# wangyunpeng139/3_ORB_SLAM3_SelfNote

Measured on AMD Instinct MI355X. Metric: frames/sec ORB extract+match, 752x480, higher is better.
Workload: dtype u8; 1 GPU; BASELINE configs[2]: extract + SearchByProjection match, 1000x1000 candidates, synthetic frame stream; image=752x480, nfeatures=1000, nlevels=8, batch=256, distinct_frames_per_gpu=2048, streams=4

## Files before the change

### 3_orb_slam3_selfnote_amd/csrc/orb_kernels.h

```cpp
#pragma once
#include <hip/hip_runtime.h>
#include <type_traits>
#include "orb_common.h"
#include "orb_fast_score.h"
#include "orb_sincos.h"

#define WAVE 64

__constant__ __attribute__((aligned(16))) int8_t c_pattern[1024] = {
#include "../../include/orb_pattern_data.inc"
};

struct DiscTab { uint32_t w[64][6]; };
constexpr DiscTab make_disc_tab() {
  DiscTab t{};
  const int umax[16] = {15, 15, 15, 15, 14, 14, 14, 13, 13, 12, 11, 10, 9, 8, 6, 3};
  int n = 0;
  for (int v = -15; v <= 15; v++) {
    const int d = umax[v < 0 ? -v : v];
    for (int u = -d; u <= d; u++) {
      const int lane = n & 63, k = n >> 6;
      t.w[lane][k >> 2] |= (uint32_t)(uint8_t)(int8_t)u << (8 * (k & 3));
      t.w[lane][3 + (k >> 2)] |= (uint32_t)(uint8_t)(int8_t)v << (8 * (k & 3));
      n++;
    }
  }
  return t;
}
__constant__ __attribute__((aligned(16))) DiscTab c_disc = make_disc_tab();

__device__ __forceinline__ int reflect101(int p, int n) {
  if (n == 1) return 0;
  while (p < 0 || p >= n) p = p < 0 ? -p : 2 * (n - 1) - p;
  return p;
}

__device__ __forceinline__ const uint8_t *level_plane(const FrameParams &P, int frame, int level, int &pitch) {
  if (level == 0) {
    pitch = (int)P.img0_stride;
    return P.img0 + (size_t)frame * P.img0_frame_stride;
  }
  pitch = P.geom[level].pitch;
  return P.pyr + (size_t)frame * P.pyr_fs + P.geom[level].off;
}

__device__ __forceinline__ void xcd_map(int nitems, uint32_t magic, int nframes, int &frame, int &item) {
  const unsigned b = blockIdx.x;
  const unsigned full = (unsigned)(nframes & ~7);
  const unsigned nfull = full * (unsigned)nitems;
  const bool inFull = b < nfull;
  const unsigned q = inFull ? (b >> 3) : (b - nfull);
  unsigned g = __umulhi(q, magic);
  unsigned r = q - g * (unsigned)nitems;
  if (r >= (unsigned)nitems) { g++; r -= (unsigned)nitems; }
  frame = (int)(inFull ? (b & 7u) + 8u * g : full + g);
  item = (int)r;
}

template <int CTRL, int ROWMASK>
__device__ __forceinline__ int dpp_or_zero(int v) { return __builtin_amdgcn_update_dpp(0, v, CTRL, ROWMASK, 0xf, false); }
__device__ __forceinline__ uint32_t mul24(uint32_t a, uint32_t u) {
  uint32_t d;
  asm("v_mul_u32_u24 %0, %1, %2" : "=v"(d) : "s"(u), "v"(a));
  return d;
}
__device__ __forceinline__ uint32_t mul24_vv(uint32_t a, uint32_t b) { return __umul24(a, b); }

__device__ __forceinline__ int wave_sum_i32(int v) {
  v += dpp_or_zero<0x111, 0xf>(v);
  v += dpp_or_zero<0x112, 0xf>(v);
  v += dpp_or_zero<0x114, 0xf>(v);
  v += dpp_or_zero<0x118, 0xf>(v);
  v += dpp_or_zero<0x142, 0xa>(v);
  v += dpp_or_zero<0x143, 0xc>(v);
  return __builtin_amdgcn_readlane(v, 63);
}

__device__ __forceinline__ uint32_t wave_incl_scan(uint32_t x) {
  int v = (int)x;
  v += dpp_or_zero<0x111, 0xf>(v);
  v += dpp_or_zero<0x112, 0xf>(v);
  v += dpp_or_zero<0x114, 0xf>(v);
  v += dpp_or_zero<0x118, 0xf>(v);
  v += dpp_or_zero<0x142, 0xa>(v);
  v += dpp_or_zero<0x143, 0xc>(v);
  return (uint32_t)v;
}

template <int NT>
__device__ uint32_t lds_excl_scan(uint32_t *a, int n, uint32_t *sw) {
  const int tid = threadIdx.x, lane = tid & 63, wid = tid >> 6;
  constexpr int NW = NT / 64;
  uint32_t carry = 0;
  for (int base = 0; base < n; base += NT) {
    int i = base + tid;
    uint32_t v = i < n ? a[i] : 0u;
    uint32_t inc = wave_incl_scan(v);
    if (lane == 63) sw[wid] = inc;
    __syncthreads();
    const uint32_t wsum = lane < NW ? sw[lane] : 0u;
    const uint32_t wincl = wave_incl_scan(wsum);
    const int widu = __builtin_amdgcn_readfirstlane(wid);
    const uint32_t woff = (uint32_t)__builtin_amdgcn_readlane((int)(wincl - wsum), widu);
    const uint32_t tot = (uint32_t)__builtin_amdgcn_readlane((int)wincl, NW - 1);
    if (i < n) a[i] = carry + woff + inc - v;
    carry += tot;
    __syncthreads();
  }
  return carry;
}

#define RESIZE_ROWS_MAX 16
#define RESIZE_MAXSRC 32
__global__ __launch_bounds__(256) void k_resize(FrameParams P, int level, int smemRowBytes, int tPitch, int maxSrc) {
  extern __shared__ __align__(16) uint8_t smem_rs[];
  const LevelGeom G = P.geom[level];
  const LevelGeom Gs = P.geom[level - 1];
  const int tid = threadIdx.x;
  int frame, rowTile;
  xcd_map((G.h + G.resizeRows - 1) / G.resizeRows, G.rowTileMagic, P.nframes, frame, rowTile);
  const int dy0 = rowTile * G.resizeRows;
  const int nrows = min(G.resizeRows, G.h - dy0);
  int spitch;
  const uint8_t *src = level_plane(P, frame, level - 1, spitch);
  uint8_t *dstplane = P.pyr + (size_t)frame * P.pyr_fs + G.off;
  const int wq = (G.w + 3) & ~3, qw = wq >> 2;
  __shared__ int2 sY[RESIZE_ROWS_MAX];
  if (tid < nrows) sY[tid] = P.ytab[G.ytabBase + dy0 + tid];

  if (tPitch > 0) {
    const int syFirst = min(max(P.ytab[G.ytabBase + dy0].x, 0), Gs.h - 1);
    const int syLast = min(max(P.ytab[G.ytabBase + dy0 + nrows - 1].x + 1, 0), Gs.h - 1);
    const int nsrc = min(syLast - syFirst + 1, maxSrc);
    uint8_t *sRows = smem_rs;
    uint8_t *sT = sRows + (size_t)maxSrc * smemRowBytes;
    uint4 *sRowRec = reinterpret_cast<uint4 *>(sT + (((size_t)maxSrc * tPitch + 15) & ~(size_t)15));
    const int4 *xtab4 = reinterpret_cast<const int4 *>(P.xtab + G.xtabBase);
    int4 xtPre[2];
#pragma unroll
    for (int k = 0; k < 2; k++) { const int p = tid + 256 * k; xtPre[k] = 2 * p < wq ? xtab4[p] : make_int4(0, 0, 0, 0); }
    const bool aligned = ((((uintptr_t)src) | (uintptr_t)spitch) & 3u) == 0;
    const uint8_t *src0 = src + (size_t)syFirst * spitch;
    if (aligned) {
      const int cpr = smemRowBytes >> 4, nfull = Gs.w >> 4;
      const float inv_cpr = 1.0f / (float)cpr;
      for (int idx = tid; idx < cpr * nsrc; idx += 256) {
        const int r = (int)(((float)idx + 0.5f) * inv_cpr), c = idx - (int)mul24((uint32_t)r, (uint32_t)cpr);
        if (c < nfull)
          __builtin_amdgcn_global_load_lds((const __attribute__((address_space(1))) void *)(src0 + (mul24((uint32_t)r, (uint32_t)spitch) + 16u * (uint32_t)c)),
                                           (__attribute__((address_space(3))) void *)(sRows + (size_t)(idx - (tid & 63)) * 16), 16, 0, 0);
      }
      const int ndw = (Gs.w + 3) >> 2, d0 = 4 * nfull, ntail = ndw - d0;
      const bool lastRowPartial = (Gs.w & 3) != 0;
      for (int idx = tid; idx < ntail * nsrc; idx += 256) {
        const int r = idx / ntail, d = d0 + (idx - r * ntail);
        const uint8_t *rowp = src0 + mul24((uint32_t)r, (uint32_t)spitch);
        uint32_t v;
        if (lastRowPartial && d == ndw - 1 && syFirst + r == Gs.h - 1 && spitch < 4 * ndw) {
          v = 0;
          for (int b = 0; 4 * d + b < Gs.w; b++) v |= (uint32_t)rowp[4 * d + b] << (8 * b);
        } else {
          v = *reinterpret_cast<const uint32_t *>(rowp + 4 * d);
        }
        *reinterpret_cast<uint32_t *>(sRows + mul24((uint32_t)r, (uint32_t)smemRowBytes) + 4 * d) = v;
      }
    } else {
      const float inv_w = 1.0f / (float)Gs.w;
      for (int idx = tid; idx < Gs.w * nsrc; idx += 256) {
        const int r = (int)(((float)idx + 0.5f) * inv_w), c = idx - (int)mul24((uint32_t)r, (uint32_t)Gs.w);
        sRows[mul24((uint32_t)r, (uint32_t)smemRowBytes) + c] = src0[mul24((uint32_t)r, (uint32_t)spitch) + c];
      }
    }
    if (tid < nrows) {
      const int2 yt = P.ytab[G.ytabBase + dy0 + tid];
      const int sy0 = min(max(yt.x, 0), Gs.h - 1), sy1 = min(max(yt.x + 1, 0), Gs.h - 1);
      sRowRec[tid] = make_uint4((uint32_t)((sy0 - syFirst) * tPitch), (uint32_t)((sy1 - syFirst) * tPitch), (uint32_t)yt.y, (uint32_t)((dy0 + tid) * G.pitch));
    }
    __syncthreads();
    typedef unsigned short u16x2 __attribute__((ext_vector_type(2)));
    auto dot2 = [](uint32_t pix, uint32_t coef) -> uint32_t {
      u16x2 x, y;
      __builtin_memcpy(&x, &pix, 4); __builtin_memcpy(&y, &coef, 4);
      return __builtin_amdgcn_udot2(x, y, 0u, false);
    };
    int trip = 0;
    for (int p = tid; 2 * p < wq; p += 256, trip++) {
      const int4 xt = trip == 0 ? xtPre[0] : trip == 1 ? xtPre[1] : xtab4[p];
      const uint32_t base = (uint32_t)xt.x & ~3u, oA = (uint32_t)xt.x & 3u, oB = (uint32_t)xt.z - base;
      const uint32_t selA = 0x0c000c00u | oA | ((oA + 1u) << 16), selB = 0x0c000c00u | oB | ((oB + 1u) << 16);
      const uint32_t kA = (uint32_t)xt.y << 4, kB = (uint32_t)xt.w << 4;
      const uint8_t *sp = sRows + base;
      uint8_t *tp = sT + 4 * p;
      for (int r = 0; r < nsrc; r += 4) {
        uint32_t lo[4], hi[4];
#pragma unroll
        for (int k = 0; k < 4; k++) {
          const uint32_t *q = reinterpret_cast<const uint32_t *>(sp + min(r + k, nsrc - 1) * smemRowBytes);
          lo[k] = q[0]; hi[k] = q[1];
        }
#pragma unroll
        for (int k = 0; k < 4; k++)
          if (r + k < nsrc) {
            const uint32_t vA = dot2(__builtin_amdgcn_perm(hi[k], lo[k], selA), kA), vB = dot2(__builtin_amdgcn_perm(hi[k], lo[k], selB), kB);
            *reinterpret_cast<uint32_t *>(tp + (r + k) * tPitch) = __builtin_amdgcn_perm(vB, vA, 0x06050201u);
          }
      }
    }
    __syncthreads();
    for (int ry = tid >> 5; ry < nrows; ry += 8) {
      const uint4 rec = sRowRec[ry];
      const uint32_t b0 = rec.z & 0xffffu, b1 = rec.z >> 16;
      const uint8_t *T0 = sT + rec.x, *T1 = sT + rec.y;
      uint8_t *dst = dstplane + rec.w;
      for (int qx = tid & 31; qx < qw; qx += 32) {
        const uint2 t0 = *reinterpret_cast<const uint2 *>(T0 + 8 * qx), t1 = *reinterpret_cast<const uint2 *>(T1 + 8 * qx);
        const uint32_t u0[4] = {t0.x & 0xffffu, t0.x >> 16, t0.y & 0xffffu, t0.y >> 16};
        const uint32_t u1[4] = {t1.x & 0xffffu, t1.x >> 16, t1.y & 0xffffu, t1.y >> 16};
        uint32_t packed = 0;
#pragma unroll
        for (int j = 0; j < 4; j++) {
          const uint32_t v = ((mul24_vv(b0, u0[j]) >> 16) + (mul24_vv(b1, u1[j]) >> 16) + 2) >> 2;
          packed |= v << (8 * j);
        }
        const int dx0 = 4 * qx;
        if (dx0 + 3 < G.w) *reinterpret_cast<uint32_t *>(dst + dx0) = packed;
        else for (int j = 0; j < 4 && dx0 + j < G.w; j++) dst[dx0 + j] = (uint8_t)(packed >> (8 * j));
      }
    }
    return;
  }

  int2 *sX = reinterpret_cast<int2 *>(smem_rs);
  for (int i = tid; i < wq; i += 256) sX[i] = P.xtab[G.xtabBase + i];
  __syncthreads();
  const float inv_qw = 1.0f / (float)qw;
  for (int q = tid; q < qw * nrows; q += 256) {
    const int ry = (int)(((float)q + 0.5f) * inv_qw), dx0 = (q - (int)mul24((uint32_t)ry, (uint32_t)qw)) * 4, dy = dy0 + ry;
    const int2 yt = sY[ry];
    const int sy0 = min(max(yt.x, 0), Gs.h - 1), sy1 = min(max(yt.x + 1, 0), Gs.h - 1);
    const int b0 = yt.y & 0xffff, b1 = (yt.y >> 16) & 0xffff;
    const uint8_t *S0 = src + mul24((uint32_t)sy0, (uint32_t)spitch), *S1 = src + mul24((uint32_t)sy1, (uint32_t)spitch);
    uint32_t packed = 0;
#pragma unroll
    for (int j = 0; j < 4; j++) {
      const int2 xt = sX[dx0 + j];
      const int sx = xt.x, sx1 = min(sx + 1, Gs.w - 1);
      const int a0 = xt.y & 0xffff, a1 = (xt.y >> 16) & 0xffff;
      const int r0 = S0[sx] * a0 + S0[sx1] * a1;
      const int r1 = S1[sx] * a0 + S1[sx1] * a1;
      const int v = (((b0 * (r0 >> 4)) >> 16) + ((b1 * (r1 >> 4)) >> 16) + 2) >> 2;
      packed |= (uint32_t)v << (8 * j);
    }
    uint8_t *dst = dstplane + mul24((uint32_t)dy, (uint32_t)G.pitch);
    if (dx0 + 3 < G.w) *reinterpret_cast<uint32_t *>(dst + dx0) = packed;
    else for (int j = 0; j < 4 && dx0 + j < G.w; j++) dst[dx0 + j] = (uint8_t)(packed >> (8 * j));
  }
}

__global__ __launch_bounds__(CHAIN_NT) void k_pyramid_chain(FrameParams P) {
  extern __shared__ __align__(16) uint8_t smem_ch[];
  const int tid = threadIdx.x, lane = tid & 63, wid = tid >> 6;
  constexpr int NW = CHAIN_NT / 64;
  const int ntile = (int)gridDim.x / P.nframes;
  const int frame = (int)blockIdx.x / ntile, tile = (int)blockIdx.x - frame * ntile;
  __shared__ ChainTile T;
  static_assert(sizeof(ChainTile) % 4 == 0 && sizeof(ChainTile) / 4 <= CHAIN_NT, "one dword per thread");
  if (tid < (int)(sizeof(ChainTile) / 4)) reinterpret_cast<uint32_t *>(&T)[tid] = reinterpret_cast<const uint32_t *>(&P.chain[tile])[tid];
  __syncthreads();
  const int L = T.level;
  uint8_t *buf[2] = {smem_ch, smem_ch + P.chainBuf0};
  int2 *sTab = reinterpret_cast<int2 *>(smem_ch + P.chainBuf0 + P.chainBuf1);
  {
    int off = 0;
    for (int l = 1; l <= L; l++) {
      const LevelGeom &G = P.geom[l];
      for (int i = tid; i < T.w[l] + T.h[l]; i += CHAIN_NT)
        sTab[off + i] = i < T.w[l] ? P.xtab[G.xtabBase + T.x[l] + i] : P.ytab[G.ytabBase + T.y[l] + (i - T.w[l])];
      off += T.w[l] + T.h[l];
    }
  }
  {
    const uint8_t *img = P.img0 + (size_t)frame * P.img0_frame_stride + (size_t)T.y[0] * P.img0_stride + T.x[0];
    const int rw = T.w[0], rh = T.h[0];
    for (int r = wid; r < rh; r += NW)
      for (int c = lane; c < rw; c += 64) buf[0][r * rw + c] = img[(size_t)r * P.img0_stride + c];
  }
  __syncthreads();
  int toff = 0;
  for (int l = 1; l <= L; l++) {
    const LevelGeom &G = P.geom[l];
    const LevelGeom &Gs = P.geom[l - 1];
    const int rw = T.w[l], rh = T.h[l], sw = T.w[l - 1], sx0 = T.x[l - 1], sy0 = T.y[l - 1];
    const uint8_t *S = buf[(l - 1) & 1];
    uint8_t *D = buf[l & 1];
    const int2 *sX = sTab + toff, *sY = sX + rw;
    toff += rw + rh;
    uint8_t *plane = P.pyr + (size_t)frame * P.pyr_fs + G.off + (size_t)T.y[l] * G.pitch + T.x[l];
    const float inv_rw = 1.0f / (float)rw;
    for (int idx = tid; idx < rw * rh; idx += CHAIN_NT) {
      const int ry = (int)(((float)idx + 0.5f) * inv_rw), rx = idx - ry * rw;
      const int2 xt = sX[rx], yt = sY[ry];
      const int sx = xt.x, sx1 = min(sx + 1, Gs.w - 1);
      const int sya = min(max(yt.x, 0), Gs.h - 1), syb = min(max(yt.x + 1, 0), Gs.h - 1);
      const int a0 = xt.y & 0xffff, a1 = (xt.y >> 16) & 0xffff, b0 = yt.y & 0xffff, b1 = (yt.y >> 16) & 0xffff;
      const uint8_t *S0 = S + (sya - sy0) * sw - sx0, *S1 = S + (syb - sy0) * sw - sx0;
      const int r0 = S0[sx] * a0 + S0[sx1] * a1;
      const int r1 = S1[sx] * a0 + S1[sx1] * a1;
      const int v = (((b0 * (r0 >> 4)) >> 16) + ((b1 * (r1 >> 4)) >> 16) + 2) >> 2;
      if (l == L) plane[(size_t)ry * G.pitch + rx] = (uint8_t)v;
      else D[idx] = (uint8_t)v;
    }
    __syncthreads();
  }
}

__device__ __forceinline__ int lane_rank(unsigned long long b) {
  return (int)__builtin_amdgcn_mbcnt_hi((uint32_t)(b >> 32), __builtin_amdgcn_mbcnt_lo((uint32_t)b, 0u));
}

__device__ __forceinline__ int fast_compass_sign(const uint8_t *c, int t) {
  constexpr int Pt = FAST_TILE_PITCH;
  const int v = c[0];
  const uint16_t p0 = c[3 * Pt], p4 = c[3], p8 = c[-3 * Pt], p12 = c[-3];
  const int D = (int)(uint16_t)max((uint16_t)min(p0, p8), (uint16_t)min(p4, p12));
  const int B = (int)(uint16_t)min((uint16_t)max(p0, p8), (uint16_t)max(p4, p12));
  return (D - (v - t)) | ((v + t) - B);
}

#ifndef FAST_NT
#define FAST_NT 256
#endif
#define FAST_QUEUE 128
#ifndef FAST_LIST
#define FAST_LIST 384
#endif
static_assert(FAST_NT == 4 * WAVE, "k_fast gives each cell of a 2 x 2 group a wavefront of its own");
static_assert(FAST_LIST % WAVE == 0, "pass 3 reads the corner list 64 entries at a time, all inside the list");
static_assert((FAST_TILE_ROWS * FAST_TILE_PITCH) % 16 == 0, "the score plane is cleared in 16-byte stores");
static_assert(FAST_TILE_ROWS * FAST_TILE_PITCH <= 65536, "queue entries are 16-bit tile offsets");
#if defined(FAST_STAMPS) || defined(OCT_STAMPS)
__device__ unsigned int *g_fast_stamps;
#endif
#ifdef FAST_STAMPS
#define FSTAMP(i) do { const long long t_ = __builtin_readcyclecounter(); if (threadIdx.x == 0 && g_fast_stamps) g_fast_stamps[(size_t)blockIdx.x * 8 + (i)] = (unsigned int)(t_ - ft0); ft0 = t_; } while (0)
#else
#define FSTAMP(i) do {} while (0)
#endif
__device__ __forceinline__ void wave_lds_order() {
  __builtin_amdgcn_wave_barrier();
  asm volatile("" ::: "memory");
}
__global__ __launch_bounds__(FAST_NT) void k_fast(FrameParams P) {
#ifdef FAST_STAMPS
  long long ft0 = __builtin_readcyclecounter();
#endif
  __shared__ __align__(16) uint8_t sTile[FAST_TILE_ROWS * FAST_TILE_PITCH];
  __shared__ __align__(16) uint8_t sS[FAST_TILE_ROWS * FAST_TILE_PITCH];
  __shared__ uint16_t sQ[4 * FAST_QUEUE];
  __shared__ uint16_t sL[4 * FAST_LIST];
  const int tid = threadIdx.x, lane = tid & 63;
  int groupId, frame;
  xcd_map(P.totalGroups, P.magicGroups, P.nframes, frame, groupId);
  const uint4 gr = reinterpret_cast<const uint4 *>(P.groups)[groupId];
  const int firstCell = (int)gr.x, gx = (int)(gr.y & 0xffu), gy = (int)((gr.y >> 8) & 0xffu), gStride = (int)(gr.y >> 16);
  const int tileX = (int)(gr.z & 0xffffu), tileY = (int)(gr.z >> 16);
  const int gtw = (int)(gr.w & 0xffu), gth = (int)((gr.w >> 8) & 0xffu), level = (int)((gr.w >> 16) & 0xffu);
  const bool gvalid = (gr.w >> 24) != 0u;
  const int ax = tileX & ~3;
  if (gvalid) {
    const uint4 r1f = reinterpret_cast<const uint4 *>(P.cells)[2 * firstCell + 1];
    int pitch;
    const uint8_t *img;
    if (level == 0) { pitch = (int)P.img0_stride; img = P.img0 + (size_t)frame * P.img0_frame_stride; }
    else { pitch = (int)r1f.y; img = P.pyr + (size_t)frame * P.pyr_fs + (((size_t)r1f.w << 32) | r1f.z); }
    const bool aligned = ((((uintptr_t)img) | (uintptr_t)pitch) & 3u) == 0;
    if (aligned) {
      const int nch = 5 * gth;
      const uint8_t *img0 = img + mul24((uint32_t)tileY, (uint32_t)pitch) + ax;
      for (int idx = tid; idx < nch; idx += FAST_NT) {
// ... 1157 lines not shown
```

### 3_orb_slam3_selfnote_amd/csrc/orbhip.hip

```cpp
#include <hip/hip_runtime.h>
#include <math.h>
#include <stdio.h>
#include <stdlib.h>
#include <string.h>
#include <string>
#include <vector>
#include <algorithm>
#include <type_traits>
#include <mutex>
#include <chrono>

#include "../../include/orbhip.h"
#include "orb_kernels.h"
#include "orb_match_kernels.h"
#include "orb_match_mfma.h"
#include "orb_project_kernels.h"
#include "orb_stereo_kernels.h"

static_assert(sizeof(orbx_keypoint_t) == 28, "cv::KeyPoint layout");
static_assert(sizeof(KpOut) == 28, "cv::KeyPoint layout");

namespace {

inline int cv_round(double v) { return (int)lrint(v); }
// ... 479 lines not shown
          ChainTile T;
          memset(&T, 0, sizeof(T));
          T.level = (uint16_t)L;
          int x0 = tx, x1 = std::min(tx + CHAIN_TILE, g[L].w) - 1, y0 = ty, y1 = std::min(ty + CHAIN_TILE, g[L].h) - 1;
          size_t tab = 0;
          for (int l = L; l >= 0; l--) {
            T.x[l] = (uint16_t)x0; T.y[l] = (uint16_t)y0; T.w[l] = (uint16_t)(x1 - x0 + 1); T.h[l] = (uint16_t)(y1 - y0 + 1);
            const size_t area = (size_t)T.w[l] * T.h[l];
            if (l < L) { if (l & 1) b1 = std::max(b1, area); else b0 = std::max(b0, area); }
            if (l == 0) break;
            tab += (size_t)T.w[l] + T.h[l];
            const int sw = g[l - 1].w, sh = g[l - 1].h;
            const int2 *xt = &xtab[g[l].xtabBase], *yt = &ytab[g[l].ytabBase];
            int nx0 = sw, nx1 = 0, ny0 = sh, ny1 = 0;
            for (int x = x0; x <= x1; x++) { nx0 = std::min(nx0, xt[x].x); nx1 = std::max(nx1, std::min(xt[x].x + 1, sw - 1)); }
            for (int y = y0; y <= y1; y++) {
              ny0 = std::min(ny0, std::min(std::max(yt[y].x, 0), sh - 1));
              ny1 = std::max(ny1, std::min(std::max(yt[y].x + 1, 0), sh - 1));
            }
            x0 = nx0; x1 = nx1; y0 = ny0; y1 = ny1;
          }
          tabMax = std::max(tabMax, tab);
          tilesC.push_back(T);
        }
    b0 = align_up(b0, 16); b1 = align_up(b1, 16);
    const size_t lds = b0 + b1 + sizeof(int2) * tabMax;
    h->chainTiles = 0;
    if (!tilesC.empty() && lds <= 64 * 1024 && b1 <= 16384 && b0 <= 65536 && tilesC.size() < 65536) {
      bool ok = true;
      for (const ChainTile &T : tilesC)
        for (int l = 1; l <= T.level; l++) ok = ok && (size_t)T.w[l] * T.h[l] < 16384;
      if (ok) {
        XCHECK(h, h->d_chain.reserve(sizeof(ChainTile) * tilesC.size()));
        XCHECK(h, copy_on(h->stream, h->d_chain.p, tilesC.data(), sizeof(ChainTile) * tilesC.size(), hipMemcpyHostToDevice));
        h->chainTiles = (int)tilesC.size(); h->chainBuf0 = (int)b0; h->chainBuf1 = (int)b1; h->chainLds = lds;
      }
    }
  }
  int maxCells = 1;
  for (int l = 0; l < nl; l++) maxCells = std::max(maxCells, g[l].nCols * g[l].nRows);
  size_t lds = 72 * (size_t)octCap + 128;
  if (lds > 160 * 1024 - 256) { h->err = "nfeatures too large for the LDS-resident octree"; return ORBX_E_ARG; }
  h->octCellsLds = lds + 4 * ((size_t)maxCells + 1) <= 96 * 1024;
  if (h->octCellsLds) lds += 4 * ((size_t)maxCells + 1);
  h->octLds = lds;
  if (lds > ORB_LDS_LIMIT) { h->err = "octree LDS state exceeds 160 KiB"; return ORBX_E_ARG; }
  h->rows = rows;
  h->cols = cols;
  h->max_batch = max_batch;
  h->have_last = false;
  return h->maxKeypoints;
}

void orbx_set_profiling(orbx_t *h, int enable) {
  if (!h) return;
  h->profiling = enable != 0;
  h->prof_head = 0;
  h->stage_valid = false;
  if (h->profiling && !h->ev_ok) {
    (void)hipSetDevice(h->device);
    bool ok = true;
    for (auto &set : h->ev)
      for (auto &e : set) ok = ok && hipEventCreate(&e) == hipSuccess;
    h->ev_ok = ok;
  }
}

int orbx_get_stage_ms(orbx_t *h, float *ms, int cap) {
  if (!h || !ms || !h->profiling || !h->ev_ok || !h->stage_valid || h->prof_head <= 0) return 0;
  const int nb = std::min(h->prof_head, PROF_DEPTH), n = std::min(cap, 5);
  if (hipEventSynchronize(h->ev[(h->prof_head - 1) % PROF_DEPTH][5]) != hipSuccess) return 0;
  for (int i = 0; i < n; i++) ms[i] = 0.f;
  for (int b = 0; b < nb; b++) {
    const int slot = (h->prof_head - 1 - b) % PROF_DEPTH;
    for (int i = 0; i < n; i++) {
      float t = 0;
      if (hipEventElapsedTime(&t, h->ev[slot][i], h->ev[slot][i + 1]) != hipSuccess) return 0;
      ms[i] += t / (float)nb;
    }
  }
  return n;
}

int orbx_extract_batch_device(orbx_t *h, const uint8_t *d_images, int rows, int cols, size_t stride, size_t frame_stride,
                              int nframes, int lap0, int lap1, orbx_keypoint_t *d_kps, uint8_t *d_desc, int32_t *d_counts,
                              int cap, void *stream_) {
  if (!h) return ORBX_E_ARG;
  if (!d_images || rows <= 0 || cols <= 0 || nframes <= 0) return ORBX_E_EMPTY;
  if (!d_kps || !d_desc || !d_counts || cap <= 0 || stride < (size_t)cols) return ORBX_E_ARG;
  int rc = orbx_configure(h, rows, cols, std::max(nframes, h->rows == rows && h->cols == cols ? h->max_batch : 1));
  if (rc < 0) return rc;
  if (cap < h->maxKeypoints) { h->err = "cap below orbx_configure()'s bound"; return ORBX_E_CAP; }
  XCHECK(h, hipSetDevice(h->device));
  hipStream_t s = (hipStream_t)stream_;
  FrameParams P;
  memset(&P, 0, sizeof(P));
  for (int l = 0; l < h->nlevels; l++) P.geom[l] = h->geom[l];
  P.nlevels = h->nlevels;
  P.nframes = nframes;
  P.iniTh = h->iniThFAST;
  P.minTh = h->minThFAST;
  P.lap0 = lap0;
  P.lap1 = lap1;
  P.img0 = d_images;
  P.img0_stride = stride;
  P.img0_frame_stride = frame_stride;
  P.pyr = (uint8_t *)h->d_pyr.p;       P.pyr_fs = h->pyr_fs;
  P.blur = (uint8_t *)h->d_blur.p;     P.blur_fs = h->blur_fs;
  P.cellCnt = (uint32_t *)h->d_cellCnt.p; P.cell_fs = h->cell_fs;
  P.slots = (uint32_t *)h->d_slots.p;  P.slot_fs = h->slot_fs;
  P.cand = (uint32_t *)h->d_cand.p;    P.cand_fs = h->cand_fs;
  P.knode = (uint16_t *)h->d_knode.p;
  P.lkp = (uint32_t *)h->d_lkp.p;      P.lkp_fs = h->lkp_fs;
  P.lrank = (uint16_t *)h->d_lrank.p;
  P.lcnt = (int32_t *)h->d_lcnt.p;
  P.candCnt = (int32_t *)h->d_candCnt.p;
  P.xtab = (const int2 *)h->d_xtab.p;
  P.ytab = (const int2 *)h->d_ytab.p;
  P.disc = (const int8_t *)h->d_disc.p;
  P.totalTiles = h->totalTiles;
  P.totalCells = h->totalCells;
  P.cells = (const uint32_t *)h->d_cells.p;
  P.groups = (const uint32_t *)h->d_groups.p;
  P.totalGroups = h->totalGroups;
  P.magicGroups = magic_div((uint32_t)std::max(h->totalGroups, 1));
  P.tiles = (const uint32_t *)h->d_tiles.p;
  P.magicCells = magic_div((uint32_t)std::max(h->totalCells, 1));
  P.magicTiles = magic_div((uint32_t)std::max(h->totalTiles, 1));
  const bool wide = (long long)h->nlevels * nframes <= 32;
  const int describeGroups = wide ? ORB_DESCRIBE_GROUPS(h->totalKp, 1) : ORB_DESCRIBE_GROUPS(h->totalKp, ORB_DESCRIBE_K);
  P.magicKpBlk = magic_div((uint32_t)describeGroups);
  P.totalKp = h->totalKp;
  P.octCap = h->octCap;
  P.chain = (const ChainTile *)h->d_chain.p; P.chainBuf0 = h->chainBuf0; P.chainBuf1 = h->chainBuf1;
  P.out_kps = d_kps;
  P.out_desc = d_desc;
  P.out_counts = d_counts;
  P.cap = cap;
  const bool prof = h->profiling && h->ev_ok;
  hipEvent_t *pev = h->ev[h->prof_head % PROF_DEPTH];
  if (prof) XCHECK(h, hipEventRecord(pev[0], s));
  const bool printForms = getenv("ORBHIP_PRINT_EXTRACT_FORMS") != nullptr;
  std::string pyrForm = h->nlevels == 1 ? "none" : "";
  if (wide && h->chainTiles > 0) { hipLaunchKernelGGL(k_pyramid_chain, dim3(h->chainTiles * nframes), dim3(CHAIN_NT), h->chainLds, s, P); pyrForm = "chain"; }
  else
  for (int l = 1; l < h->nlevels; l++) {
    const LevelGeom &G = h->geom[l], &Gs = h->geom[l - 1];
    const int rowBytes = (int)align_up((size_t)Gs.w + 4, 16);
    const int wq = (G.w + 3) & ~3;
    const int tPitch2 = (int)align_up((size_t)wq * 2, 8);
    const size_t lds2 = (size_t)G.resizeSrcRows * rowBytes + align_up((size_t)G.resizeSrcRows * tPitch2, 16) + 16 * RESIZE_ROWS_MAX;
    const bool twoPass = G.resizeSrcRows <= RESIZE_MAXSRC && (double)Gs.w / G.w < 3.0 && lds2 <= ORB_LDS_LIMIT - 1024;
    const int tPitch = twoPass ? tPitch2 : 0;
    const size_t lds = twoPass ? lds2 : (size_t)wq * 8;
    hipLaunchKernelGGL(k_resize, dim3(((G.h + G.resizeRows - 1) / G.resizeRows) * nframes), dim3(256), lds, s, P, l, rowBytes, tPitch, G.resizeSrcRows);
    if (printForms) pyrForm += std::string(l > 1 ? "," : "") + (!twoPass ? "1p" : G.resizeRows == 16 ? "2p16" : "2p8");
  }
  if (prof) XCHECK(h, hipEventRecord(pev[1], s));
  if (h->totalGroups > 0) hipLaunchKernelGGL(k_fast, dim3(h->totalGroups * nframes), dim3(FAST_NT), 0, s, P);
  if (prof) XCHECK(h, hipEventRecord(pev[2], s));
  if (wide) {
    if (h->octCellsLds) hipLaunchKernelGGL((k_octree<1024, true>), dim3(h->nlevels * nframes), dim3(1024), h->octLds, s, P, (uint32_t *)h->d_cellOff.p);
    else hipLaunchKernelGGL((k_octree<1024, false>), dim3(h->nlevels * nframes), dim3(1024), h->octLds, s, P, (uint32_t *)h->d_cellOff.p);
  } else {
    if (h->octCellsLds) hipLaunchKernelGGL((k_octree<256, true>), dim3(h->nlevels * nframes), dim3(256), h->octLds, s, P, (uint32_t *)h->d_cellOff.p);
    else hipLaunchKernelGGL((k_octree<256, false>), dim3(h->nlevels * nframes), dim3(256), h->octLds, s, P, (uint32_t *)h->d_cellOff.p);
  }
  if (prof) XCHECK(h, hipEventRecord(pev[3], s));
  hipLaunchKernelGGL(k_blur, dim3(h->totalTiles * nframes), dim3(256), 0, s, P);
  if (prof) XCHECK(h, hipEventRecord(pev[4], s));
  if (wide) hipLaunchKernelGGL(k_describe<1>, dim3(describeGroups * nframes), dim3(256), 0, s, P);
  else hipLaunchKernelGGL(k_describe<ORB_DESCRIBE_K>, dim3(describeGroups * nframes), dim3(256), 0, s, P);
  if (prof) { XCHECK(h, hipEventRecord(pev[5], s)); h->prof_head++; h->stage_valid = true; }
  XCHECK(h, hipGetLastError());
  if (printForms) {
    int aligned0 = 0;
    for (int f = 0; f < nframes; f++) aligned0 += (((uintptr_t)(d_images + (size_t)f * frame_stride) | (uintptr_t)stride) & 3u) == 0;
    const LevelGeom &G0 = h->geom[0];
    const int blur0dma = G0.w >= 160 && G0.h >= 40 && (G0.w & 15) == 0 ? aligned0 : 0;
    fprintf(stderr, "orbhip: extract nframes %d pyramid %s octree %d/%s aligned0 %d blur0dma %d describe %d\n", nframes, pyrForm.c_str(), wide ? 1024 : 256,
            h->octCellsLds ? "lds" : "global", aligned0, blur0dma, wide ? 1 : ORB_DESCRIBE_K);
  }
  h->last = P;
  h->have_last = true;
  if (!h->in_capture) {
    if (!h->last_done) XCHECK(h, hipEventCreateWithFlags(&h->last_done, hipEventDisableTiming));
    XCHECK(h, hipEventRecord(h->last_done, s));
    h->last_pending = true;
  }
  return 0;
}

int orbx_extract(orbx_t *h, const uint8_t *image, int rows, int cols, size_t stride, int lap0, int lap1,
                 orbx_keypoint_t *keypoints, uint8_t *descriptors, int cap, int *n_out) {
  if (!h) return ORBX_E_ARG;
  if (n_out) *n_out = 0;
  if (!image || rows <= 0 || cols <= 0) return ORBX_E_EMPTY;
  if (stride < (size_t)cols || !n_out) return ORBX_E_ARG;
  int rc = orbx_configure(h, rows, cols, h->rows == rows && h->cols == cols ? h->max_batch : 1);
  if (rc < 0) return rc;
  const int icap = h->maxKeypoints;
  const size_t dstride = align_up((size_t)cols, 64);
  XCHECK(h, hipSetDevice(h->device));
  XCHECK(h, h->d_img.reserve(dstride * rows));
  const size_t in_bytes = dstride * rows, kp_bytes = sizeof(orbx_keypoint_t) * (size_t)icap, de_bytes = 32 * (size_t)icap;
  const size_t kp_off = 64, de_off = kp_off + align_up(kp_bytes, 64), out_bytes = de_off + de_bytes;
  XCHECK(h, h->d_okps.reserve(out_bytes));
  if (h->pin_in_bytes < in_bytes) {
    if (h->pin_in) (void)hipHostFree(h->pin_in);
    h->pin_in = nullptr; h->pin_in_bytes = 0;
    XCHECK(h, hipHostMalloc(&h->pin_in, in_bytes, hipHostMallocDefault));
    h->pin_in_bytes = in_bytes;
  }
  if (h->pin_out_bytes < out_bytes) {
    if (h->pin_out) (void)hipHostFree(h->pin_out);
    h->pin_out = nullptr; h->pin_out_bytes = 0;
    XCHECK(h, hipHostMalloc(&h->pin_out, out_bytes, hipHostMallocDefault));
    h->pin_out_bytes = out_bytes;
  }
  const auto t0 = std::chrono::steady_clock::now();
  for (int y = 0; y < rows; y++) memcpy((uint8_t *)h->pin_in + (size_t)y * dstride, image + (size_t)y * stride, (size_t)cols);
  const auto t1 = std::chrono::steady_clock::now();
  uint8_t *po = (uint8_t *)h->pin_out;
  auto enqueue = [&]() -> int {
    XCHECK(h, hipMemcpyAsync(h->d_img.p, h->pin_in, in_bytes, hipMemcpyHostToDevice, h->stream));
    uint8_t *dout = (uint8_t *)h->d_okps.p;
    const int r = orbx_extract_batch_device(h, (const uint8_t *)h->d_img.p, rows, cols, dstride, dstride * rows, 1, lap0, lap1,
                                            (orbx_keypoint_t *)(dout + kp_off), dout + de_off, (int32_t *)dout, icap, h->stream);
    if (r < 0) return r;
    XCHECK(h, hipMemcpyAsync(po, dout, out_bytes, hipMemcpyDeviceToHost, h->stream));
    return 0;
  };
  bool launched = false;
  if (h->graph_ok && !h->profiling) {
    auto &K = h->graph_key;
    const bool same = h->graph && K.rows == rows && K.cols == cols && K.lap0 == lap0 && K.lap1 == lap1 && K.icap == icap && K.pin_in == h->pin_in &&
                      K.pin_out == h->pin_out && K.d_img == h->d_img.p && K.d_okps == h->d_okps.p && K.d_pyr == h->d_pyr.p;
    if (!same) {
      if (h->graph) { (void)hipGraphExecDestroy(h->graph); h->graph = nullptr; }
      hipGraph_t g = nullptr;
      if (hipStreamBeginCapture(h->stream, hipStreamCaptureModeThreadLocal) == hipSuccess) {
        h->in_capture = true;
        const int r = enqueue();
        h->in_capture = false;
        const hipError_t e = hipStreamEndCapture(h->stream, &g);
        if (r == 0 && e == hipSuccess && g && hipGraphInstantiate(&h->graph, g, nullptr, nullptr, 0) == hipSuccess) {
          K.rows = rows; K.cols = cols; K.lap0 = lap0; K.lap1 = lap1; K.icap = icap; K.pin_in = h->pin_in; K.pin_out = h->pin_out;
          K.d_img = h->d_img.p; K.d_okps = h->d_okps.p; K.d_pyr = h->d_pyr.p;
        } else {
          h->graph = nullptr;
          h->graph_ok = false;
          (void)hipGetLastError();
        }
        if (g) (void)hipGraphDestroy(g);
      } else {
        h->graph_ok = false;
        (void)hipGetLastError();
      }
    }
    if (h->graph) {
      XCHECK(h, hipGraphLaunch(h->graph, h->stream));
      launched = true;
    }
  }
  if (!launched) { rc = enqueue(); if (rc < 0) return rc; }
  const auto t2 = std::chrono::steady_clock::now();
  XCHECK(h, hipStreamSynchronize(h->stream));
  const auto t3 = std::chrono::steady_clock::now();
  h->last_pending = false;
  int32_t counts[2];
  memcpy(counts, po, sizeof(counts));
  *n_out = counts[0];
  if (counts[0] > cap) return ORBX_E_CAP;
  if (counts[0] > 0) {
    if (!keypoints || !descriptors) return ORBX_E_ARG;
    memcpy(keypoints, po + kp_off, sizeof(orbx_keypoint_t) * (size_t)counts[0]);
    memcpy(descriptors, po + de_off, 32 * (size_t)counts[0]);
  }
  const auto t4 = std::chrono::steady_clock::now();
  auto us = [](std::chrono::steady_clock::time_point a, std::chrono::steady_clock::time_point b) { return std::chrono::duration<float, std::micro>(b - a).count(); };
  h->host_us[0] = us(t0, t1); h->host_us[1] = us(t1, t2); h->host_us[2] = us(t2, t3); h->host_us[3] = us(t3, t4);
  return counts[1];
}

int orbx_get_host_us(const orbx_t *h, float *us, int cap) {
  if (!h || !us || cap < 4) return ORBX_E_ARG;
  for (int i = 0; i < 4; i++) us[i] = h->host_us[i];
  return 4;
}

int orbx_cvt_color_gray_device(const uint8_t *d_src, int rows, int cols, size_t src_stride, int channels, int rgb_order, uint8_t *d_dst,
                               size_t dst_stride, void *stream) {
  if (!d_src || !d_dst || rows <= 0 || cols <= 0 || (channels != 3 && channels != 4) || src_stride < (size_t)cols * channels || dst_stride < (size_t)cols)
    return ORBX_E_ARG;
  hipLaunchKernelGGL(k_cvt_gray, dim3((cols + 1023) / 1024, rows), dim3(256), 0, (hipStream_t)stream, d_src, rows, cols, src_stride, channels,
                     rgb_order ? 1 : 0, d_dst, dst_stride);
  return hipGetLastError() == hipSuccess ? 0 : ORBX_E_HIP;
}

int orbx_cvt_color_gray(orbx_t *h, const uint8_t *src, int rows, int cols, size_t src_stride, int channels, int rgb_order, uint8_t *dst,
                        size_t dst_stride) {
  if (!h || !src || !dst || rows <= 0 || cols <= 0 || (channels != 3 && channels != 4) || src_stride < (size_t)cols * channels || dst_stride < (size_t)cols)
    return ORBX_E_ARG;
  XCHECK(h, hipSetDevice(h->device));
  const size_t sbytes = (size_t)cols * channels, dpitch = align_up((size_t)cols, 64);
  XCHECK(h, h->stereo[0].reserve(sbytes * rows));
  XCHECK(h, h->stereo[1].reserve(dpitch * rows));
  XCHECK(h, hipMemcpy2DAsync(h->stereo[0].p, sbytes, src, src_stride, sbytes, (size_t)rows, hipMemcpyHostToDevice, h->stream));
// ... 1784 lines not shown
```

Measured before the change: 283,500 frames/s.

## Fuse two-pass resize into streaming per-column vertical sweep without LDS intermediate

New measurement: 272,400 frames/s. 0.961x the previous value.

```diff
diff --git a/3_orb_slam3_selfnote_amd/csrc/orb_kernels.h b/3_orb_slam3_selfnote_amd/csrc/orb_kernels.h
--- a/3_orb_slam3_selfnote_amd/csrc/orb_kernels.h
+++ b/3_orb_slam3_selfnote_amd/csrc/orb_kernels.h
@@ -112,7 +112,12 @@
 
 #define RESIZE_ROWS_MAX 16
 #define RESIZE_MAXSRC 32
-__global__ __launch_bounds__(256) void k_resize(FrameParams P, int level, int smemRowBytes, int tPitch, int maxSrc) {
+#ifndef RESIZE_RUN_WIDE
+#define RESIZE_RUN_WIDE 8
+#endif
+__host__ __device__ inline int resize_run_rows(int qw) { return qw > 64 ? RESIZE_RUN_WIDE : 4; }
+__device__ __forceinline__ uint32_t resize_vsum(uint32_t b0, uint32_t T0, uint32_t b1, uint32_t T1) { return (mul24(T0, b0) >> 16) + (mul24(T1, b1) >> 16) + 2u; }
+__global__ __launch_bounds__(256) void k_resize(FrameParams P, int level, int smemRowBytes, int tPitch, int maxSrc, int runRows) {
   extern __shared__ __align__(16) uint8_t smem_rs[];
   const LevelGeom G = P.geom[level];
   const LevelGeom Gs = P.geom[level - 1];
@@ -133,12 +138,19 @@
     const int syLast = min(max(P.ytab[G.ytabBase + dy0 + nrows - 1].x + 1, 0), Gs.h - 1);
     const int nsrc = min(syLast - syFirst + 1, maxSrc);
     uint8_t *sRows = smem_rs;
-    uint8_t *sT = sRows + (size_t)maxSrc * smemRowBytes;
-    uint4 *sRowRec = reinterpret_cast<uint4 *>(sT + (((size_t)maxSrc * tPitch + 15) & ~(size_t)15));
+    uint4 *sRowRec = reinterpret_cast<uint4 *>(sRows + (size_t)maxSrc * smemRowBytes);
+    const int lane = tid & 63;
+    const int nchunk = (qw + 63) >> 6, nitem = ((nrows + runRows - 1) / runRows) * nchunk;
     const int4 *xtab4 = reinterpret_cast<const int4 *>(P.xtab + G.xtabBase);
-    int4 xtPre[2];
-#pragma unroll
-    for (int k = 0; k < 2; k++) { const int p = tid + 256 * k; xtPre[k] = 2 * p < wq ? xtab4[p] : make_int4(0, 0, 0, 0); }
+    int item = __builtin_amdgcn_readfirstlane(tid >> 6), run = 0, chunk = item;
+    while (chunk >= nchunk) { chunk -= nchunk; run++; }
+    int4 xtNext[2];
+    {
+      const int qx = 64 * chunk + lane;
+      const bool on = item < nitem && qx < qw;
+      xtNext[0] = on ? xtab4[2 * qx] : make_int4(0, 0, 0, 0);
+      xtNext[1] = on ? xtab4[2 * qx + 1] : make_int4(0, 0, 0, 0);
+    }
     const bool aligned = ((((uintptr_t)src) | (uintptr_t)spitch) & 3u) == 0;
     const uint8_t *src0 = src + (size_t)syFirst * spitch;
     if (aligned) {
@@ -174,7 +186,7 @@
     if (tid < nrows) {
       const int2 yt = P.ytab[G.ytabBase + dy0 + tid];
       const int sy0 = min(max(yt.x, 0), Gs.h - 1), sy1 = min(max(yt.x + 1, 0), Gs.h - 1);
-      sRowRec[tid] = make_uint4((uint32_t)((sy0 - syFirst) * tPitch), (uint32_t)((sy1 - syFirst) * tPitch), (uint32_t)yt.y, (uint32_t)((dy0 + tid) * G.pitch));
+      sRowRec[tid] = make_uint4((uint32_t)((sy0 - syFirst) * smemRowBytes), (uint32_t)((sy1 - syFirst) * smemRowBytes), (uint32_t)yt.y, (uint32_t)((dy0 + tid) * G.pitch));
     }
     __syncthreads();
     typedef unsigned short u16x2 __attribute__((ext_vector_type(2)));
@@ -183,48 +195,71 @@
       __builtin_memcpy(&x, &pix, 4); __builtin_memcpy(&y, &coef, 4);
       return __builtin_amdgcn_udot2(x, y, 0u, false);
     };
-    int trip = 0;
-    for (int p = tid; 2 * p < wq; p += 256, trip++) {
-      const int4 xt = trip == 0 ? xtPre[0] : trip == 1 ? xtPre[1] : xtab4[p];
-      const uint32_t base = (uint32_t)xt.x & ~3u, oA = (uint32_t)xt.x & 3u, oB = (uint32_t)xt.z - base;
-      const uint32_t selA = 0x0c000c00u | oA | ((oA + 1u) << 16), selB = 0x0c000c00u | oB | ((oB + 1u) << 16);
-      const uint32_t kA = (uint32_t)xt.y << 4, kB = (uint32_t)xt.w << 4;
-      const uint8_t *sp = sRows + base;
-      uint8_t *tp = sT + 4 * p;
-      for (int r = 0; r < nsrc; r += 4) {
-        uint32_t lo[4], hi[4];
-#pragma unroll
-        for (int k = 0; k < 4; k++) {
-          const uint32_t *q = reinterpret_cast<const uint32_t *>(sp + min(r + k, nsrc - 1) * smemRowBytes);
-          lo[k] = q[0]; hi[k] = q[1];
-        }
-#pragma unroll
-        for (int k = 0; k < 4; k++)
-          if (r + k < nsrc) {
-            const uint32_t vA = dot2(__builtin_amdgcn_perm(hi[k], lo[k], selA), kA), vB = dot2(__builtin_amdgcn_perm(hi[k], lo[k], selB), kB);
-            *reinterpret_cast<uint32_t *>(tp + (r + k) * tPitch) = __builtin_amdgcn_perm(vB, vA, 0x06050201u);
-          }
-      }
-    }
-    __syncthreads();
-    for (int ry = tid >> 5; ry < nrows; ry += 8) {
-      const uint4 rec = sRowRec[ry];
-      const uint32_t b0 = rec.z & 0xffffu, b1 = rec.z >> 16;
-      const uint8_t *T0 = sT + rec.x, *T1 = sT + rec.y;
-      uint8_t *dst = dstplane + rec.w;
-      for (int qx = tid & 31; qx < qw; qx += 32) {
-        const uint2 t0 = *reinterpret_cast<const uint2 *>(T0 + 8 * qx), t1 = *reinterpret_cast<const uint2 *>(T1 + 8 * qx);
-        const uint32_t u0[4] = {t0.x & 0xffffu, t0.x >> 16, t0.y & 0xffffu, t0.y >> 16};
-        const uint32_t u1[4] = {t1.x & 0xffffu, t1.x >> 16, t1.y & 0xffffu, t1.y >> 16};
-        uint32_t packed = 0;
-#pragma unroll
-        for (int j = 0; j < 4; j++) {
-          const uint32_t v = ((mul24_vv(b0, u0[j]) >> 16) + (mul24_vv(b1, u1[j]) >> 16) + 2) >> 2;
-          packed |= v << (8 * j);
-        }
-        const int dx0 = 4 * qx;
-        if (dx0 + 3 < G.w) *reinterpret_cast<uint32_t *>(dst + dx0) = packed;
-        else for (int j = 0; j < 4 && dx0 + j < G.w; j++) dst[dx0 + j] = (uint8_t)(packed >> (8 * j));
+    const uint4 recv = sRowRec[lane & (RESIZE_ROWS_MAX - 1)];
+    const uint32_t rb = (uint32_t)smemRowBytes;
+    while (item < nitem) {
+      const int4 xt0 = xtNext[0], xt1 = xtNext[1];
+      const uint32_t dx0 = 4u * (uint32_t)(64 * chunk + lane);
+      uint8_t *dcol = dstplane + dx0;
+      const int j0 = run * runRows, j1 = min(j0 + runRows, nrows);
+      item += 4; chunk += 4;
+      while (chunk >= nchunk) { chunk -= nchunk; run++; }
+      {
+        const int qn = 64 * chunk + lane;
+        const bool on = item < nitem && qn < qw;
+        xtNext[0] = on ? xtab4[2 * qn] : make_int4(0, 0, 0, 0);
+        xtNext[1] = on ? xtab4[2 * qn + 1] : make_int4(0, 0, 0, 0);
+      }
+      const uint32_t base0 = (uint32_t)xt0.x & ~3u, base1 = (uint32_t)xt1.x & ~3u;
+      uint32_t sel[4], kc[4];
+      {
+        const uint32_t oA = (uint32_t)xt0.x & 3u, oB = (uint32_t)xt0.z - base0, oC = (uint32_t)xt1.x & 3u, oD = (uint32_t)xt1.z - base1;
+        sel[0] = 0x0c000c00u | oA | ((oA + 1u) << 16); sel[1] = 0x0c000c00u | oB | ((oB + 1u) << 16);
+        sel[2] = 0x0c000c00u | oC | ((oC + 1u) << 16); sel[3] = 0x0c000c00u | oD | ((oD + 1u) << 16);
+        kc[0] = (uint32_t)xt0.y << 4; kc[1] = (uint32_t)xt0.w << 4; kc[2] = (uint32_t)xt1.y << 4; kc[3] = (uint32_t)xt1.w << 4;
+      }
+      const uint8_t *sp0 = sRows + base0, *sp1 = sRows + base1;
+      auto load_win = [&](uint32_t ro, uint32_t (&w)[4]) __attribute__((always_inline)) {
+        const uint32_t *q0 = reinterpret_cast<const uint32_t *>(sp0 + ro), *q1 = reinterpret_cast<const uint32_t *>(sp1 + ro);
+        w[0] = q0[0]; w[1] = q0[1]; w[2] = q1[0]; w[3] = q1[1];
+      };
+      auto hsum = [&](const uint32_t (&w)[4], uint32_t (&T)[4]) __attribute__((always_inline)) {
+        const uint32_t d0 = dot2(__builtin_amdgcn_perm(w[1], w[0], sel[0]), kc[0]), d1 = dot2(__builtin_amdgcn_perm(w[1], w[0], sel[1]), kc[1]);
+        const uint32_t d2 = dot2(__builtin_amdgcn_perm(w[3], w[2], sel[2]), kc[2]), d3 = dot2(__builtin_amdgcn_perm(w[3], w[2], sel[3]), kc[3]);
+        T[0] = d0 >> 8; T[1] = d1 >> 8; T[2] = d2 >> 8; T[3] = d3 >> 8;
+      };
+      auto row_rec = [&](int j) __attribute__((always_inline)) -> uint4 {
+        if (j >= j1) return make_uint4(0xffffffffu, 0xffffffffu, 0u, 0u);
+        return make_uint4((uint32_t)__builtin_amdgcn_readlane((int)recv.x, j), (uint32_t)__builtin_amdgcn_readlane((int)recv.y, j),
+                          (uint32_t)__builtin_amdgcn_readlane((int)recv.z, j), (uint32_t)__builtin_amdgcn_readlane((int)recv.w, j));
+      };
+      auto emit = [&](const uint4 rec, const uint32_t (&T0)[4], const uint32_t (&T1)[4]) __attribute__((always_inline)) {
+        const uint32_t b0 = rec.z & 0xffffu, b1 = rec.z >> 16;
+        uint32_t sum[4];
+#pragma unroll
+        for (int k = 0; k < 4; k++) sum[k] = resize_vsum(b0, T0[k], b1, T1[k]);
+        const uint32_t packed = __builtin_amdgcn_perm((sum[2] | (sum[3] << 16)) >> 2, (sum[0] | (sum[1] << 16)) >> 2, 0x06040200u);
+        uint8_t *dst = dcol + rec.w;
+        if (dx0 + 3 < (uint32_t)G.w) *reinterpret_cast<uint32_t *>(dst) = packed;
+        else for (uint32_t k = 0; k < 4 && dx0 + k < (uint32_t)G.w; k++) dst[k] = (uint8_t)(packed >> (8 * k));
+      };
+      int j = j0;
+      uint4 rec = row_rec(j);
+      uint32_t s = rec.x;
+      const uint32_t sEnd = (uint32_t)__builtin_amdgcn_readlane((int)recv.y, j1 - 1);
+      uint32_t E[4] = {0, 0, 0, 0}, O[4] = {0, 0, 0, 0}, w[4];
+      load_win(s, w);
+      for (;;) {
+        if (rec.x == s || rec.y == s) hsum(w, E);
+        if (s < sEnd) load_win(s + rb, w);
+        while (rec.y == s) { if (rec.x == s) emit(rec, E, E); else emit(rec, O, E); rec = row_rec(++j); }
+        if (s >= sEnd) break;
+        s += rb;
+        if (rec.x == s || rec.y == s) hsum(w, O);
+        if (s < sEnd) load_win(s + rb, w);
+        while (rec.y == s) { if (rec.x == s) emit(rec, O, O); else emit(rec, E, O); rec = row_rec(++j); }
+        if (s >= sEnd) break;
+        s += rb;
       }
     }
     return;
diff --git a/3_orb_slam3_selfnote_amd/csrc/orbhip.hip b/3_orb_slam3_selfnote_amd/csrc/orbhip.hip
--- a/3_orb_slam3_selfnote_amd/csrc/orbhip.hip
+++ b/3_orb_slam3_selfnote_amd/csrc/orbhip.hip
@@ -655,8 +655,12 @@
     const size_t lds2 = (size_t)G.resizeSrcRows * rowBytes + align_up((size_t)G.resizeSrcRows * tPitch2, 16) + 16 * RESIZE_ROWS_MAX;
     const bool twoPass = G.resizeSrcRows <= RESIZE_MAXSRC && (double)Gs.w / G.w < 3.0 && lds2 <= ORB_LDS_LIMIT - 1024;
     const int tPitch = twoPass ? tPitch2 : 0;
+#ifdef RESIZE_LDS_PAD_EXPERIMENT
     const size_t lds = twoPass ? lds2 : (size_t)wq * 8;
-    hipLaunchKernelGGL(k_resize, dim3(((G.h + G.resizeRows - 1) / G.resizeRows) * nframes), dim3(256), lds, s, P, l, rowBytes, tPitch, G.resizeSrcRows);
+#else
+    const size_t lds = twoPass ? (size_t)G.resizeSrcRows * rowBytes + 16 * RESIZE_ROWS_MAX : (size_t)wq * 8;
+#endif
+    hipLaunchKernelGGL(k_resize, dim3(((G.h + G.resizeRows - 1) / G.resizeRows) * nframes), dim3(256), lds, s, P, l, rowBytes, tPitch, G.resizeSrcRows, resize_run_rows(wq >> 2));
     if (printForms) pyrForm += std::string(l > 1 ? "," : "") + (!twoPass ? "1p" : G.resizeRows == 16 ? "2p16" : "2p8");
   }
   if (prof) XCHECK(h, hipEventRecord(pev[1], s));
```
